# peterdavidfagan/mujoco_robot_environments

Measured on AMD Instinct MI355X. Metric: env steps/sec (whole node), RearrangementEnv batch=4096 at 1/2/4/8 MI355X, higher is better.
Workload: dtype f32

## Files before the change

mujoco_robot_environments_amd/csrc/mre_newton.h:

```cpp
#pragma once

namespace mre {

constexpr int NW_QUAD = 0, NW_SAT = 1, NW_CONE = 4;
constexpr int NW_LS_MAX = 20;
constexpr float NW_LS_TOL = 0.01f;
#ifndef NW_LS_REL_VALUE
#define NW_LS_REL_VALUE 1e-5f
#endif
constexpr float NW_LS_REL = NW_LS_REL_VALUE;

MRE_DEV float rdlane(float v, int lane) {
  return __builtin_bit_cast(float, __builtin_amdgcn_readlane(__builtin_bit_cast(int, v), lane));
}
MRE_DEV int uni(int v) { return __builtin_amdgcn_readfirstlane(v); }
MRE_DEV float unif(float v) {
  return __builtin_bit_cast(float, __builtin_amdgcn_readfirstlane(__builtin_bit_cast(int, v)));
}

MRE_DEV float nw_Jl(const Sm& s, int i, int h, int l, int lp, int lk) {
  const int rs = h & 0xFF, pa = (h >> 8) & 0xF, pb = (h >> 12) & 0xF;
  float j = 0.f;
  if (l < NRV) {
    if (rs != HDR_NONE) j = s.Jr[rs][l];
// ... 93 lines not shown
    const NwContact o = pyr ? nw_pyramid<FULL>(jar[i], jar[i + 1], jar[i + 2], D0, fr, hc)
                            : nw_contact<FULL>(jar[i], jar[i + 1], jar[i + 2], D0, D1, D2, fr, fr * mu_scale, hc);
    cost += o.cost;
    if (FULL) {
      s.frc[i] = o.f0; s.frc[i + 1] = o.f1; s.frc[i + 2] = o.f2;
      const int rs = s.con_rslot[l];
      if (rs != HDR_NONE) { s.frc_r[rs] = o.f0; s.frc_r[rs + 1] = o.f1; s.frc_r[rs + 2] = o.f2; }
      s.rstate[i] = s.rstate[i + 1] = s.rstate[i + 2] = (uint8_t)o.st;
      if (o.st == NW_CONE) {
#pragma unroll
        for (int k = 0; k < 6; k++) s.hc[l][k] = hc[k];
      }
    }
  }
  return wave_sum(cost);
}

struct NwMasks { unsigned long long sc, cq, cc; };
MRE_DEV bool operator==(const NwMasks& a, const NwMasks& b) { return a.sc == b.sc && a.cq == b.cq && a.cc == b.cc; }
MRE_DEV NwMasks nw_masks(const Sm& s, int l, int nscalar, int ncon) {
  NwMasks m;
  const int st_s = l < nscalar ? s.rstate[l] : NW_SAT;
  const int st_c = l < ncon ? s.rstate[nscalar + 3 * l] : NW_SAT;
  m.sc = __ballot(st_s == NW_QUAD);
  m.cq = __ballot(st_c == NW_QUAD);
  m.cc = __ballot(st_c == NW_CONE);
  return m;
}

MRE_DEV float nw_JTf(const Sm& s, int l, int lp, int lk, int nscalar) {
  float acc = 0.f;
  if (l < NRV) {
    const int n = s.nrrow;
    for (int rs = 0; rs < n; rs++) acc = fmaf(s.Jr[rs][l], s.frc_r[rs], acc);
  } else if (l < NV && lp < s.nprops) {
    const int n = s.ccount[lp];
    for (int t = 0; t < n; t++) {
      const int e = s.clist[lp][t], c = e & 0x7F;
      const float* J = (e & 0x80) ? s.JpB[3 * s.con_bslot[c]] : s.JpA[3 * c];
      const float* f = &s.frc[nscalar + 3 * c];
      acc = fmaf(J[lk], f[0], acc);
      acc = fmaf(J[6 + lk], f[1], acc);
      acc = fmaf(J[12 + lk], f[2], acc);
    }
  }
  return acc;
}

MRE_DEV void nw_rank1(float (&hh)[NV], float t, float J, bool has_r, int pa, int pb) {
  if (has_r) {
#pragma unroll
    for (int c = 0; c < NRV; c++) hh[c] = fmaf(t, rdlane(J, c), hh[c]);
  }
#pragma unroll
  for (int p = 0; p < NPROP; p++) {
    if (pa == p || pb == p) {
#pragma unroll
      for (int k = 0; k < 6; k++) hh[NRV + 6 * p + k] = fmaf(t, rdlane(J, NRV + 6 * p + k), hh[NRV + 6 * p + k]);
    }
  }
}

template <int HI, int LO>
MRE_DEV void nw_elim_update(float (&hh)[NV], float u) {
  constexpr int n = HI - LO + 1;
  if constexpr (n > 0) {
#pragma unroll
    for (int g0 = 0; g0 < n; g0 += 8) {
      float t[8];
#pragma unroll
      for (int q = 0; q < 8; q++)
        if (g0 + q < n) t[q] = rdlane(u, HI - g0 - q);
      __builtin_amdgcn_sched_barrier(0);
#pragma unroll
      for (int q = 0; q < 8; q++)
        if (g0 + q < n) hh[HI - g0 - q] = fmaf(-u, t[q], hh[HI - g0 - q]);
// ... 79 lines not shown
  c.lp = (l >= NRV && l < NV) ? (l - NRV) / 6 : -1;
  c.lk = (l >= NRV && l < NV) ? (l - NRV) % 6 : 0;
  c.lact = l < NRV || (c.lp >= 0 && c.lp < s.nprops);
  c.mdiag = c.lp >= 0 ? (c.lk < 3 ? s.prop_mass[c.lp] : s.prop_inertia[c.lp][c.lk - 3]) : 0.f;
  c.mu_scale = __builtin_amdgcn_rsqf(fmaxf(M->impratio, kMinVal));
  float msum = M->M0_diag_robot_sum;
  for (int p = 0; p < s.nprops; p++)
    msum += 3.f * s.prop_mass[p] + s.prop_inertia[p][0] + s.prop_inertia[p][1] + s.prop_inertia[p][2];
  c.scale = 1.0f / msum;
  return c;
}

template <bool PYR>
MRE_DEV float nw_update_gradient(Sm& s, int l, const NwLane& c, int nscalar, int ncon) {
  const float sc = nw_update<true, PYR>(s, l, nscalar, ncon, c.mu_scale, s.jar);
  MRE_SYNC();
  const float qc = nw_JTf(s, l, c.lp, c.lk, nscalar);
  const bool on = l < NV && c.lact;
  const float fs = on ? s.qfrc_smooth[l] : 0.f, as = on ? s.qacc_smooth[l] : 0.f;
  const float qa = on ? s.qacc[l] : 0.f, Ma = on ? s.nw_Ma[l] : 0.f;
  if (l < NVP) {
    s.qfrc_con[l] = on ? qc : 0.f;
    s.nw_grad[l] = on ? Ma - fs - qc : 0.f;
  }
  const float cost = sc + wave_sum(0.5f * (Ma - fs) * (qa - as));
  MRE_SYNC();
  return cost;
}

template <bool PYR>
MRE_DEV float nw_setup_impl(ModelP M, Sm& s, int l) {
  const NwLane c = nw_lane(M, s, l);
  const int nefc = s.nefc, ncon = s.ncon, nscalar = 7 + s.nl;
  for (int e = l; e < NRV * MD_LD; e += 64) (&s.Md[0][0])[e] = 0.f;
  MRE_SYNC();
  for (int e = l; e < NMR; e += 64) {
    const int i = M->M_i[e], j = M->M_j[e];
    const float v = s.qM[e];
    s.Md[i][j] = v; s.Md[j][i] = v;
  }
  MRE_SYNC();
  const bool on = l < NV && c.lact;
  const float fs = on ? s.qfrc_smooth[l] : 0.f, as = on ? s.qacc_smooth[l] : 0.f;
  float qa = on ? s.qacc[l] : 0.f;
  float Ma = on ? nw_mulM(s, l, c.mdiag, s.qacc) : 0.f;
  for (int i = l; i < nefc; i += 64) {
    const float aref = s.efc_aref[i];
    float d1, d2;
    row_dot2(s, i, s.qacc, s.qacc_smooth, d1, d2);
    s.jar[i] = d1 - aref;
    s.jv[i] = d2 - aref;
  }
  MRE_SYNC();
  const float gauss = wave_sum(0.5f * (Ma - fs) * (qa - as));
  const float cost_ws = gauss + nw_update<false, PYR>(s, l, nscalar, ncon, c.mu_scale, s.jar);
  const float cost_sm = nw_update<false, PYR>(s, l, nscalar, ncon, c.mu_scale, s.jv);
  if (cost_ws > cost_sm || !(cost_ws == cost_ws)) {
    qa = as; Ma = fs;
    for (int i = l; i < nefc; i += 64) s.jar[i] = s.jv[i];
  }
  if (l < NVP) { s.qacc[l] = qa; s.nw_Ma[l] = Ma; }
  MRE_SYNC();
  return nw_update_gradient<PYR>(s, l, c, nscalar, ncon);
}
MRE_PHASE_FN float nw_setup(ModelP M, Sm& s, int l) { return nw_setup_impl<false>(M, s, l); }
MRE_PHASE_FN float nw_setup_pyramidal(ModelP M, Sm& s, int l) { return nw_setup_impl<true>(M, s, l); }

MRE_PHASE_FN void nw_direction(ModelP M, Sm& s, int l) {
  MRE_DBG_T0();
  const NwLane c = nw_lane(M, s, l);
  const int nefc = s.nefc, nscalar = 7 + s.nl, nprops = s.nprops;
  const int lp = c.lp, lk = c.lk;
  float hh[NV];
#pragma unroll
  for (int k = 0; k < NV; k++) {
    float v = 0.f;
    if (k < NRV) { if (l < NRV) v = s.Md[l][k]; }
    else if (l == k) v = c.lact ? c.mdiag : 1.0f;
    hh[k] = v;
  }
  MRE_DBG_STAMP(4, 0);
#if defined(MRE_PHASE_STAMPS) && MRE_PHASE_STAMPS == 5
  {
    int nc_ = 0, nq_ = 0;
    for (int r0 = 0; r0 < nefc; r0 += 64) {
      const int st_ = r0 + l < nefc ? (int)s.rstate[r0 + l] : NW_SAT;
      nc_ += __popcll(__ballot(st_ == NW_CONE)); nq_ += __popcll(__ballot(st_ == NW_QUAD));
    }
    if (threadIdx.x == 0) { dbg_acc[2] += (unsigned long long)nc_ << 4; dbg_acc[3] += (unsigned long long)nq_ << 4; }
  }
#endif
  typedef float v4f __attribute__((ext_vector_type(4)));
  v4f c00 = {0.f, 0.f, 0.f, 0.f}, c10 = c00, c11 = c00, c20 = c00, c21 = c00, c22 = c00;
  {
    const int g = l >> 4, m16 = l & 15;
    const char* const sb = reinterpret_cast<const char*>(&s);
    const unsigned zoff = (unsigned)offsetof(Sm, zrow), jr0 = (unsigned)offsetof(Sm, Jr);
    const unsigned sh = m16 < 12 ? 16u * (unsigned)(m16 / 6) : 0u;
    const unsigned lo = 4u * (unsigned)(m16 % 6), lr = 4u * (unsigned)m16;
    auto ldw = [&](unsigned off) { return *reinterpret_cast<const float*>(sb + off); };
    auto meta = [&](int r0, int& ii, int& st, int& h, float& R, uint2& d) {
      const int i = r0 + g;
      ii = i < nefc ? i : 0;
      st = i < nefc ? (int)s.rstate[ii] : NW_SAT;
      h = s.hdr[ii];
      R = s.efc_R[ii];
      d = *reinterpret_cast<const uint2*>(&s.jdesc[ii][0]);
    };
    auto gather = [&](int h, uint2 d, float& w0, float& w1, float& w2) {
      const int rs = h & 0xFF;
      w0 = ldw((rs != HDR_NONE ? jr0 + 60u * (unsigned)rs : zoff) + lr);
      w1 = ldw(((d.x >> sh) & 0xFFFFu) + lo);
      w2 = nprops > 2 ? ldw(((d.y >> sh) & 0xFFFFu) + lo) : 0.f;
    };
    static_assert(sizeof(s.Jr[0]) == 60 && sizeof(s.JpA[0]) == 24 && sizeof(s.JpB[0]) == 24, "row strides of the gathers");
    struct Meta { int ii, st, h; float R; uint2 d; };
    auto chunk = [&](const Meta& cur, Meta& nxt, int r0) {
      const int ii = cur.ii, h = cur.h, st = cur.st;
      const uint2 d = cur.d;
      const bool quad = st == NW_QUAD, cone = st == NW_CONE;
      const float D = quad ? __builtin_amdgcn_rcpf(cur.R) : 0.f;
      if (r0 + 4 < nefc) meta(r0 + 4, nxt.ii, nxt.st, nxt.h, nxt.R, nxt.d);
      float v0, v1, v2, a0, a1, a2;
      if (__any(cone)) {
        const int cr = ii - nscalar;
        const int k = cone ? cr % 3 : 0;
        const int i0 = ii - k, i1 = cone ? i0 + 1 : ii, i2 = cone ? i0 + 2 : ii;
        float x0, x1, x2, y0, y1, y2, z0, z1, z2;
        gather(s.hdr[i0], *reinterpret_cast<const uint2*>(&s.jdesc[i0][0]), x0, x1, x2);
        gather(s.hdr[i1], *reinterpret_cast<const uint2*>(&s.jdesc[i1][0]), y0, y1, y2);
        gather(s.hdr[i2], *reinterpret_cast<const uint2*>(&s.jdesc[i2][0]), z0, z1, z2);
        const float* hcp = s.hc[cone ? cr / 3 : 0];
        const float H0 = k == 0 ? hcp[0] : (k == 1 ? hcp[1] : hcp[2]);
        const float H1 = k == 0 ? hcp[1] : (k == 1 ? hcp[3] : hcp[4]);
        const float H2 = k == 0 ? hcp[2] : (k == 1 ? hcp[4] : hcp[5]);
        v0 = k == 0 ? x0 : (k == 1 ? y0 : z0);
        v1 = k == 0 ? x1 : (k == 1 ? y1 : z1);
        v2 = k == 0 ? x2 : (k == 1 ? y2 : z2);
        a0 = cone ? H0 * x0 + H1 * y0 + H2 * z0 : v0 * D;
        a1 = cone ? H0 * x1 + H1 * y1 + H2 * z1 : v1 * D;
        a2 = cone ? H0 * x2 + H1 * y2 + H2 * z2 : v2 * D;
      } else {
        gather(h, d, v0, v1, v2);
        a0 = v0 * D; a1 = v1 * D; a2 = v2 * D;
      }
      c00 = __builtin_amdgcn_mfma_f32_16x16x4f32(a0, v0, c00, 0, 0, 0);
      c10 = __builtin_amdgcn_mfma_f32_16x16x4f32(a1, v0, c10, 0, 0, 0);
      c11 = __builtin_amdgcn_mfma_f32_16x16x4f32(a1, v1, c11, 0, 0, 0);
      if (nprops > 2) {
        c20 = __builtin_amdgcn_mfma_f32_16x16x4f32(a2, v0, c20, 0, 0, 0);
        c21 = __builtin_amdgcn_mfma_f32_16x16x4f32(a2, v1, c21, 0, 0, 0);
        c22 = __builtin_amdgcn_mfma_f32_16x16x4f32(a2, v2, c22, 0, 0, 0);
      }
    };
    Meta mA, mB;
    meta(0, mA.ii, mA.st, mA.h, mA.R, mA.d);
    mB = mA;
    for (int r0 = 0; r0 < nefc; r0 += 8) {
      chunk(mA, mB, r0);
      if (r0 + 4 < nefc) chunk(mB, mA, r0 + 4);
    }
    MRE_DBG_STAMP(4, 1);
    float* T = s.W;
    constexpr int TS = 17;
    const int mytile = l < NRV ? 0 : (l < NRV + 12 ? 1 : (l < NV ? 2 : -1));
    const int mym = l < NRV ? l : (l < NRV + 12 ? l - NRV : l - NRV - 12);
    auto spill = [&](const v4f& cv, int off) {
#pragma unroll
      for (int v = 0; v < 4; v++) T[off + (4 * g + v) * TS + m16] = cv[v];
    };
#define NW_TILE(OFF, TI, TJ, BI, NI, BJ, NJ)                                                   \
    if (mytile == TI) {                                                                        \
      _Pragma("unroll") for (int n = 0; n < NJ; n++) hh[BJ + n] += T[OFF + mym * TS + n];      \
    }                                                                                          \
    if (TI != TJ && mytile == TJ) {                                                            \
      _Pragma("unroll") for (int q = 0; q < NI; q++) hh[BI + q] += T[OFF + q * TS + mym];      \
    }
    constexpr int T2 = 16 * TS;
    static_assert(2 * T2 <= NV * (NV + 1) / 2, "two tiles fit the factor's storage");
    spill(c00, 0); spill(c10, T2);
    MRE_SYNC();
    NW_TILE(0, 0, 0, 0, NRV, 0, NRV)
    if (nprops > 0) { NW_TILE(T2, 1, 0, NRV, 12, 0, NRV) }
    MRE_SYNC();
    if (nprops > 0) {
      spill(c11, 0); spill(c20, T2);
      MRE_SYNC();
      NW_TILE(0, 1, 1, NRV, 12, NRV, 12)
      if (nprops > 2) { NW_TILE(T2, 2, 0, NRV + 12, 12, 0, NRV) }
      MRE_SYNC();
// ... 68 lines not shown
  float g = gin;
  const float dinv = on ? 1.0f / s.W[l * (l + 1) / 2 + l] : 1.0f;
  float y = 0.f;
  for (int k = nva - 1; k >= 0; k--) {
    const float yk = rdlane(g * dinv, k);
    const float w = (l < k) ? s.W[k * (k + 1) / 2 + l] : 0.f;
    g = fmaf(-w, yk, g);
    y = (l == k) ? yk : y;
  }
  const int base = l < NV ? l * (l + 1) / 2 : 0;
  for (int j = 0; j < nva; j++) {
    const float cw = (j < l && l < NV) ? s.W[base + j] : 0.f;
    const float xj = rdlane(y * dinv, j);
    y = fmaf(-cw, xj, y);
  }
  const float x = on ? y * dinv : 0.f;
  if (l < NVP) s.nw_search[l] = -x;
  const float dec = wave_sum(gin * x);
  if (l == 0) s.scratch[2] = dec;
  MRE_SYNC();
}

template <bool PYR>
MRE_DEV float nw_search_move_impl(ModelP M, Sm& s, int l) {
  MRE_DBG_T0();
  const NwLane c = nw_lane(M, s, l);
  const int nefc = s.nefc, ncon = s.ncon, nscalar = 7 + s.nl;
  const float tol = M->tolerance, mu_scale = c.mu_scale;
  const bool on = l < NV && c.lact;
  const float fs = on ? s.qfrc_smooth[l] : 0.f, as = on ? s.qacc_smooth[l] : 0.f;
  float qa = on ? s.qacc[l] : 0.f, Ma = on ? s.nw_Ma[l] : 0.f;
  const float sv = on ? s.nw_search[l] : 0.f;
  const float Mv = on ? nw_mulM(s, l, c.mdiag, s.nw_search) : 0.f;
  for (int i = l; i < nefc; i += 64) s.jv[i] = row_dot(s, i, s.nw_search);
  MRE_SYNC();
  MRE_DBG_STAMP(7, 0);
  const float snorm = sqrtf(wave_sum(sv * sv));
  float alpha = 0.f;
#if defined(MRE_PHASE_STAMPS) && MRE_PHASE_STAMPS == 7
  int dbg_nev = 0;
#endif
  if (snorm >= kMinVal) {
    const float gtol_abs = tol * NW_LS_TOL * snorm / c.scale;
    float g0 = 0.5f * (Ma - fs) * (qa - as), g1 = sv * (Ma - fs), g2 = 0.5f * sv * Mv;
    wave_sum3(g0, g1, g2);
    float sq0 = 0.f, sq1 = 0.f, sq2 = 0.f, sj = 0.f, svv = 0.f;
    const bool s_on = l < nscalar, s_eq = l < 7;
    if (s_on) {
      const float D = 1.0f / s.efc_R[l];
      sj = s.jar[l]; svv = s.jv[l];
      sq0 = 0.5f * D * sj * sj; sq1 = D * sj * svv; sq2 = 0.5f * D * svv * svv;
    }
    float cq0 = 0.f, cq1 = 0.f, cq2 = 0.f, U0 = 0.f, V0 = 0.f, UU = 0.f, UV = 0.f, VV = 0.f, Dm = 0.f, mu = 0.f;
    const bool c_on = l < ncon;
    constexpr bool pyr = PYR;
    float pe0 = 0.f, pe1 = 0.f, pe2 = 0.f, pe3 = 0.f, pv0 = 0.f, pv1 = 0.f, pv2 = 0.f, pv3 = 0.f, pD = 0.f;
    if (c_on && pyr) {
      const int i = nscalar + 3 * l;
      const float fr = s.con_fric[l];
      const float j0 = s.jar[i], j1 = fr * s.jar[i + 1], j2 = fr * s.jar[i + 2];
      const float v0 = s.jv[i], v1 = fr * s.jv[i + 1], v2 = fr * s.jv[i + 2];
      pe0 = j0 + j1; pe1 = j0 - j1; pe2 = j0 + j2; pe3 = j0 - j2;
      pv0 = v0 + v1; pv1 = v0 - v1; pv2 = v0 + v2; pv3 = v0 - v2;
      pD = 1.0f / s.efc_R[i];
    }
    if (c_on && !pyr) {
      const int i = nscalar + 3 * l;
// ... 250 lines not shown
        const double Dm = D[0] / fmax(mu * mu * (1.0 + mu * mu), 1e-15), NT = Nn - mu * T, iT = 1.0 / T;
        o[0] = -Dm * NT * mu;
        o[1] = -o[0] * iT * U1 * fr;
        o[2] = -o[0] * iT * U2 * fr;
        const double a = mu * Nn * iT * iT * iT, dgn = mu * mu - mu * Nn * iT;
        o[3] = Dm * mu * mu;
        o[4] = Dm * mu * fr * (-mu * U1 * iT);
        o[5] = Dm * mu * fr * (-mu * U2 * iT);
        o[6] = Dm * fr * fr * (a * U1 * U1 + dgn);
        o[7] = Dm * fr * fr * (a * U1 * U2);
        o[8] = Dm * fr * fr * (a * U2 * U2 + dgn);
      }
    }
  }
  if (l < nscalar) {
    double jar = -(double)s.efc_aref[l];
#pragma unroll
    for (int j = 0; j < NRV; j++) jar += (double)s.Jr[l][j] * (double)s.qacc[j];
    const bool act = l < 7 || s.rstate[l] == NW_QUAD;
    const double D = act ? rcp_d((double)s.efc_R[l]) : 0.0;
    frow[l] = -D * jar;
    drow[l] = D;
  }
  MRE_SYNC();
  const int d = l < NRV ? l : 0;
  const bool row = l < NRV && (full || l >= F0);
  double hrow[NRV], g = 0.0;
#pragma unroll
  for (int j = 0; j < NRV; j++) hrow[j] = row ? (double)s.Md[d][j] : 0.0;
  if (row) {
    g = -(double)s.qfrc_smooth[d];
#pragma unroll
    for (int j = 0; j < NRV; j++) g += (double)s.Md[d][j] * (double)s.qacc[j];
    for (int r = 0; r < nscalar; r++) {
      const double jd = (double)s.Jr[r][d];
      g -= jd * frow[r];
      const double t = drow[r] * jd;
      if (full) {
#pragma unroll
        for (int j = 0; j < F0; j++) hrow[j] += t * (double)s.Jr[r][j];
      }
#pragma unroll
      for (int j = F0; j < NRV; j++) hrow[j] += t * (double)s.Jr[r][j];
    }
    for (int k = 0; k < nrc; k++) {
      const double* o = fcon + 10 * k;
      const int rs = (int)o[9];
      const double j0 = (double)s.Jr[rs][d], j1 = (double)s.Jr[rs + 1][d], j2 = (double)s.Jr[rs + 2][d];
      g -= j0 * o[0] + j1 * o[1] + j2 * o[2];
      const double t0 = j0 * o[3] + j1 * o[4] + j2 * o[5], t1 = j0 * o[4] + j1 * o[6] + j2 * o[7],
                   t2 = j0 * o[5] + j1 * o[7] + j2 * o[8];
      if (full) {
#pragma unroll
        for (int j = 0; j < F0; j++)
          hrow[j] += t0 * (double)s.Jr[rs][j] + t1 * (double)s.Jr[rs + 1][j] + t2 * (double)s.Jr[rs + 2][j];
      }
#pragma unroll
      for (int j = F0; j < NRV; j++)
        hrow[j] += t0 * (double)s.Jr[rs][j] + t1 * (double)s.Jr[rs + 1][j] + t2 * (double)s.Jr[rs + 2][j];
    }
  }
  double x = -g;
  double pinv[NRV];
#pragma unroll
  for (int k = 0; k < NRV; k++) pinv[k] = 1.0;
  if (full) {
#pragma unroll
    for (int k = 0; k < F0; k++) {
      pinv[k] = rcp_d(rdlane_d(hrow[k], k));
      const double xk = rdlane_d(x, k);
      const double mlt = (l > k && l < NRV) ? hrow[k] * pinv[k] : 0.0;
#pragma unroll
      for (int j = k + 1; j < NRV; j++) hrow[j] -= mlt * rdlane_d(hrow[j], k);
      x -= mlt * xk;
    }
  }
#pragma unroll
  for (int k = F0; k < NRV; k++) {
    pinv[k] = rcp_d(rdlane_d(hrow[k], k));
    if (k == NRV - 1) break;
    const double xk = rdlane_d(x, k);
    const double mlt = (l > k && l < NRV) ? hrow[k] * pinv[k] : 0.0;
#pragma unroll
    for (int j = k + 1; j < NRV; j++) hrow[j] -= mlt * rdlane_d(hrow[j], k);
    x -= mlt * xk;
  }
#pragma unroll
  for (int k = NRV - 1; k >= F0; k--) {
    const double xk = rdlane_d(x, k) * pinv[k];
    if (l == k) x = xk;
    else if (l < k && row) x -= hrow[k] * xk;
  }
// ... 19 lines not shown
```

mujoco_robot_environments_amd/csrc/mre_solver.h:

```cpp
#pragma once

namespace mre {

constexpr int HDR_NONE = 0xFF;
constexpr int BLK_NONE = 0x7F;
constexpr int SCHED_NONE = 0xFF;
constexpr int TAB_OFF = MAXBLK * 5;
constexpr int TAB_ZEROS = 48;
static_assert(TAB_BYTES == 8 * (TAB_OFF + 1) + 4 * TAB_ZEROS, "operand table size");

#ifndef MRE_NEWTON
MRE_DEV void build_schedule(ModelP M, Sm& s);
#endif
MRE_DEV constexpr int cube_pair_bit(int p, int q) {
  const int a = p < q ? p : q, b = p < q ? q : p;
  return a == 0 ? b - 1 : (a == 1 ? b + 1 : 5);
}

MRE_DEV float prop_invM(const Sm& s, int p, int k) {
  return 1.0f / ((k < 3) ? s.prop_mass[p] : s.prop_inertia[p][k - 3]);
}

MRE_DEV void geom_pose(ModelP M, const Sm& s, int g, float* p, float* R, float* size,
                       float* rbound) {
// ... 150 lines not shown
  }
}

MRE_DEV float impedance(const float* solimp, float pos, float margin) {
  const float dmin = clampf(solimp[0], 0.0001f, 0.9999f), dmax = clampf(solimp[1], 0.0001f, 0.9999f);
  const float width = fmaxf(solimp[2], kMinVal), mid = clampf(solimp[3], 0.0001f, 0.9999f);
  const float power = fmaxf(solimp[4], 1.0f);
  if (dmin == dmax) return 0.5f * (dmin + dmax);
  const float x = fabsf((pos - margin) / width);
  if (x >= 1.0f) return dmax;
  if (x <= 0.0f) return dmin;
  float y;
  if (power == 1.0f) y = x;
  else if (power == 2.0f) {
    y = (x <= mid) ? x * x / mid : 1.0f - (1.0f - x) * (1.0f - x) / (1.0f - mid);
  }
  else if (x <= mid) y = powf(x, power) / powf(mid, power - 1.0f);
  else y = 1.0f - powf(1.0f - x, power) / powf(1.0f - mid, power - 1.0f);
  return dmin + y * (dmax - dmin);
}

MRE_DEV void jac_robot(ModelP M, Sm& s, int rs, int b, const float* p, const float* ax, float sg) {
  float off[3];
  v3sub(off, p, s.com_robot);
  const int n = M->chain_len[b];
  for (int k = 0; k < n; k++) {
    const int j = M->chain_dof[b][k];
    const float* c = s.cdof[j];
    float t[3];
    v3cross(t, c, off);
    s.Jr[rs][j] += sg * (ax[0] * (c[3] + t[0]) + ax[1] * (c[4] + t[1]) + ax[2] * (c[5] + t[2]));
  }
}
MRE_DEV int row_blk(const Sm& s, int i, int& r) {
  const int ns = 7 + s.nl;
  if (i < ns) { r = i % 3; return i / 3; }
  const int cr = i - ns;
  r = cr % 3;
  return 8 + cr / 3;
}
#ifdef MRE_NEWTON
MRE_DEV float& rowR(Sm& s, int i) { return s.efc_R[i]; }
MRE_DEV float& rowB(Sm& s, int i) { return s.efc_aref[i]; }
#else
MRE_DEV float& rowR(Sm& s, int i) { int r; const int b = row_blk(s, i, r); return s.blkrec[b][r]; }
MRE_DEV float& rowB(Sm& s, int i) { int r; const int b = row_blk(s, i, r); return s.blkrec[b][3 + r]; }
MRE_DEV float& rowAinv(Sm& s, int i) { int r; const int b = row_blk(s, i, r); return s.blkrec[b][6 + r]; }
#endif

MRE_DEV float* jpA(Sm& s, int i) { return s.JpA[i - 7 - s.nl]; }
MRE_DEV const float* jpA(const Sm& s, int i) { return s.JpA[i - 7 - s.nl]; }
MRE_DEV float* jpB(Sm& s, int i) { const int cr = i - 7 - s.nl; return s.JpB[3 * s.con_bslot[cr / 3] + cr % 3]; }
MRE_DEV const float* jpB(const Sm& s, int i) { const int cr = i - 7 - s.nl; return s.JpB[3 * s.con_bslot[cr / 3] + cr % 3]; }
MRE_DEV void jac_prop(Sm& s, int i, int slot, int b, const float* p, const float* ax, float sg) {
  float off[3];
  v3sub(off, p, s.xpos[b]);
  float* J = slot == 0 ? jpA(s, i) : jpB(s, i);
  for (int k = 0; k < 3; k++) {
    J[k] = sg * ax[k];
    float axk[3] = {s.xmat[b][k], s.xmat[b][3 + k], s.xmat[b][6 + k]}, t[3];
    v3cross(t, axk, off);
    J[3 + k] = sg * v3dot(ax, t);
  }
}

MRE_DEV float row_dot(const Sm& s, int i, const float* vec) {
  const int h = s.hdr[i];
  const int rs = h & 0xFF, pa = (h >> 8) & 0xF, pb = (h >> 12) & 0xF;
  float acc = 0.f;
  if (rs != HDR_NONE)
    for (int j = 0; j < NRV; j++) acc += s.Jr[rs][j] * vec[j];
  if (pa < NPROP)
    { const float* ja = jpA(s, i); for (int k = 0; k < 6; k++) acc += ja[k] * vec[NRV + 6 * pa + k]; }
  if (pb < NPROP)
    { const float* jb = jpB(s, i); for (int k = 0; k < 6; k++) acc += jb[k] * vec[NRV + 6 * pb + k]; }
  return acc;
}

MRE_DEV void row_dot2(const Sm& s, int i, const float* v1, const float* v2, float& r1, float& r2) {
  const int h = s.hdr[i];
  const int rs = h & 0xFF, pa = (h >> 8) & 0xF, pb = (h >> 12) & 0xF;
  float a1 = 0.f, a2 = 0.f;
  if (rs != HDR_NONE)
    for (int j = 0; j < NRV; j++) { const float jv = s.Jr[rs][j]; a1 += jv * v1[j]; a2 += jv * v2[j]; }
  if (pa < NPROP) {
    const float* ja = jpA(s, i);
    for (int k = 0; k < 6; k++) { const float jv = ja[k]; a1 += jv * v1[NRV + 6 * pa + k]; a2 += jv * v2[NRV + 6 * pa + k]; }
  }
  if (pb < NPROP) {
    const float* jb = jpB(s, i);
    for (int k = 0; k < 6; k++) { const float jv = jb[k]; a1 += jv * v1[NRV + 6 * pb + k]; a2 += jv * v2[NRV + 6 * pb + k]; }
  }
  r1 = a1; r2 = a2;
}

#ifndef MRE_NEWTON
MRE_PHASE_FN void solve_robot_rows(Sm& s, int l) {
  for (int rs = l; rs < s.nrrow; rs += 64) {
    float x[NRV];
#pragma unroll
    for (int k = 0; k < NRV; k++) x[k] = s.Jr[rs][k];
    solve_robot_regs(s.qLD, s.qLDinv, x);
#pragma unroll
    for (int k = 0; k < NRV; k++) s.Br[rs][k] = x[k];
  }
  MRE_SYNC();
}

#endif

constexpr int GRIP0 = GRIP_BODY0;

MRE_PHASE_FN void assemble_constraints(ModelP M, Sm& s, int l) {
  int lim = 0, lim_side = 0;
  const auto* BR = &M->body_rec[l < NRB ? l : 0];
  const int jnt_limited = BR->jnt_limited;
  const float jnt_range[2] = {BR->jnt_range[0], BR->jnt_range[1]};
  if (l >= 1 && l < NRB && jnt_limited) {
    const double q = robot_q(s, l - 1);
    if (q - (double)jnt_range[0] < 0.0) { lim = 1; lim_side = -1; }
    else if ((double)jnt_range[1] - q < 0.0) { lim = 1; lim_side = 1; }
  }
  keep_live(jnt_range[0]); keep_live(jnt_range[1]);
  const unsigned long long limm = __ballot(lim != 0);
  const int lim_idx = __popcll(limm & ((1ull << l) - 1ull));
  if (l == 0) s.nl = __popcll(limm);
  if (lim) s.lim_info[lim_idx] = l | ((lim_side > 0 ? 1 : 0) << 8);
// ... 37 lines not shown
      s.nefc = base + 3 * kept;
      s.nrrow = base + 3 * __popcll(rmask & below);
      s.npp = __popcll(tmask & below);
      s.finger_contact = (fingm & below) != 0ull;
#ifdef MRE_NEWTON
      s.nsched = 0; s.nblk = 0;
#else
      build_schedule(M, s);
#endif
    }
  }
  MRE_SYNC();
  const int nefc = s.nefc, nl = s.nl;
  for (int e = l; e < s.nrrow * NRV; e += 64) (&s.Jr[0][0])[e] = 0.f;
#ifndef MRE_NEWTON
  for (int e = l; e < 8 * 16; e += 64) (&s.blkrec[0][0])[e] = 0.f;
#endif
  MRE_SYNC();
  for (int i = l; i < nefc; i += 64) {
    int rs = HDR_NONE, pa = 0xF, pb = 0xF;
    float pos = 0.f, margin = 0.f, diag = 0.f, imp_pos = 0.f;
    bool fric_row = false;
    float R0scale = 1.0f;
    const int eqi = i < 6 ? i / 3 : 2;
    const int limb = (i >= 7 && i < 7 + nl) ? (s.lim_info[i - 7] & 0xFF) : 0;
    const int rrec = i < 7 ? eqi : (i < 7 + nl ? ROWREC_JNT + limb : ROWREC_PAIR + s.con_pair[(i - 7 - nl) / 3]);
    const auto* RR = &M->row_rec[rrec];
    const float solref[2] = {RR->solref[0], RR->solref[1]};
    const float solimp[5] = {RR->solimp[0], RR->solimp[1], RR->solimp[2], RR->solimp[3], RR->solimp[4]};
    const float rec_margin = RR->margin, rec_gap = RR->gap, rec_friction = RR->friction, invw1 = RR->invw1, invw2 = RR->invw2;
    const float lim_range[2] = {M->body_rec[limb].jnt_range[0], M->body_rec[limb].jnt_range[1]};
    const float opt_timestep = M->opt_rec.timestep, opt_impratio = M->opt_rec.impratio;
    const int opt_cone = M->opt_rec.cone;
    if (i < 7) {
      rs = i;
      const int e = eqi;
      const auto* E = &M->eq_rec[e];
      const int b1 = E->b1, b2 = E->b2;
      const int root = E->root, pb1 = E->pb1, pb2 = E->pb2;
      const float pc[5] = {E->data[0], E->data[1], E->data[2], E->data[3], E->data[4]};
      const float q0_1 = E->qpos0_1, q0_2 = E->qpos0_2;
      const int nchain = E->root_chain_len;
      int chain[MAXCHAIN];
#pragma unroll
      for (int c = 0; c < MAXCHAIN; c++) chain[c] = E->root_chain[c];
      if (e < 2) {
        const int k = i % 3;
        const float* loc = &s.qfrc_con[16 * e];
        const float* R = s.xmat[root];
        float cp[3];
        m3mulv(cp, R, loc);
        const float rk[3] = {R[3 * k], R[3 * k + 1], R[3 * k + 2]};
        s.Jr[rs][b1 - 1] += v3dot(rk, loc + 4);
        if (pb1 >= GRIP0) s.Jr[rs][pb1 - 1] += v3dot(rk, loc + 7);
        s.Jr[rs][b2 - 1] += v3dot(rk, loc + 10);
        if (pb2 >= GRIP0) s.Jr[rs][pb2 - 1] += v3dot(rk, loc + 13);
        {
#pragma unroll
          for (int c = 0; c < MAXCHAIN; c++) {
            if (c < nchain) {
              const int j = chain[c];
              float t[3];
              v3cross(t, s.cdof[j], cp);
              s.Jr[rs][j] += sel3(t, k);
            }
          }
        }
        pos = sel3(cp, k);
        imp_pos = v3norm(cp);
        diag = invw1 + invw2;
      } else {
        const int d1 = b1 - 1, d2 = b2 - 1;
        const double dif64 = robot_q(s, d2) - (double)q0_2;
        pos = (float)(robot_q(s, d1) - (double)q0_1 -
                      ((double)pc[0] + dif64 * ((double)pc[1] + dif64 * ((double)pc[2] + dif64 * ((double)pc[3] + dif64 * (double)pc[4])))));
        const float dif = (float)dif64;
        const float deriv = pc[1] + dif * (2.f * pc[2] + dif * (3.f * pc[3] + dif * 4.f * pc[4]));
        s.Jr[rs][d1] += 1.f;
        s.Jr[rs][d2] -= deriv;
        imp_pos = pos;
        diag = invw1 + invw2;
      }
      keep_live(root); keep_live(pb1); keep_live(pb2); keep_live(nchain); keep_live(q0_1); keep_live(q0_2);
#pragma unroll
      for (int c = 0; c < 5; c++) keep_live(pc[c]);
#pragma unroll
      for (int c = 0; c < MAXCHAIN; c++) keep_live(chain[c]);
    } else if (i < 7 + nl) {
      rs = i;
      const int info = s.lim_info[i - 7], b = info & 0xFF, hi = (info >> 8) & 1;
      const double q = robot_q(s, b - 1);
      pos = (float)(hi ? ((double)lim_range[1] - q) : (q - (double)lim_range[0]));
      s.Jr[rs][b - 1] = hi ? -1.f : 1.f;
      imp_pos = pos;
      diag = invw1;
    } else {
      const int c = (i - 7 - nl) / 3, r = (i - 7 - nl) % 3;
      const int b1 = s.con_b1[c], b2 = s.con_b2[c];
      const float* ax = &s.con_frame[c][3 * r];
      const float* p = s.con_pos[c];
      const int rs0 = s.con_rslot[c];
      if (rs0 != HDR_NONE) rs = rs0 + r;
      int slot = 0;
      float dg = 0.f;
      if (b1 > 0) {
        if (b1 < NRB) { jac_robot(M, s, rs, b1, p, ax, -1.f); dg += invw1; }
        else { pa = b1 - NRB; jac_prop(s, i, slot++, b1, p, ax, -1.f); dg += 1.0f / s.prop_mass[pa]; }
      }
      if (b2 > 0) {
        if (b2 < NRB) { jac_robot(M, s, rs, b2, p, ax, 1.f); dg += invw2; }
        else {
          const int pid = b2 - NRB;
          if (slot == 0) pa = pid; else pb = pid;
          jac_prop(s, i, slot++, b2, p, ax, 1.f);
          dg += 1.0f / s.prop_mass[pid];
        }
      }
      diag = dg;
      margin = rec_margin - rec_gap;
      imp_pos = s.con_dist[c];
      if (r == 0) pos = s.con_dist[c];
      else {
        fric_row = true;
        pos = 0.f;
        R0scale = 1.0f / fmaxf(opt_impratio, kMinVal);
      }
      if (opt_cone == 0) {
        const float fr = rec_friction;
        diag = dg * (1.f + fr * fr);
        R0scale = 2.f * fr * fr / fmaxf(opt_impratio, kMinVal);
      }
    }
    keep_live(lim_range[0]); keep_live(lim_range[1]); keep_live(invw1); keep_live(invw2); keep_live(rec_friction);
    keep_live(rec_margin); keep_live(rec_gap); keep_live(opt_impratio); keep_live(opt_cone);
    s.hdr[i] = rs | (pa << 8) | (pb << 12);
    const float imp = impedance(solimp, imp_pos, margin);
    float tc = solref[0];
    const float dr = solref[1], dmax = clampf(solimp[1], 0.0001f, 0.9999f);
    float K, B;
    if (tc > 0.f) {
      tc = fmaxf(tc, 2.f * opt_timestep);
      K = 1.0f / (dmax * dmax * tc * tc * dr * dr);
      B = 2.0f / (dmax * tc);
    } else { K = -tc / (dmax * dmax); B = -dr / dmax; }
    if (fric_row) K = 0.f;
    float R = fmaxf((1.f - imp) * diag / imp, kMinVal) * R0scale;
    if (opt_cone == 0) R = fmaxf(R, kMinVal);
    const float vel = row_dot(s, i, s.qvel);
    const float efc_margin = fric_row ? 0.f : margin;
    const float aref = -B * vel - K * imp * (pos - efc_margin);
    rowR(s, i) = R; rowB(s, i) = aref;
#ifdef MRE_NEWTON
    if (i >= 7 + nl && (i - 7 - nl) % 3 == 0) s.con_fric[(i - 7 - nl) / 3] = rec_friction;
#else
    if (i >= 7 + nl && (i - 7 - nl) % 3 == 0) s.blkrec[8 + (i - 7 - nl) / 3][15] = rec_friction;
#endif
  }
  MRE_SYNC();
}

#ifndef MRE_NEWTON
MRE_PHASE_FN void assemble_blocks(ModelP M, Sm& s, int l) {
  const int nefc = s.nefc, nl = s.nl;
  for (int i = l; i < nefc; i += 64) {
    const int h = s.hdr[i];
    const int rs = h & 0xFF, pa = (h >> 8) & 0xF, pb = (h >> 12) & 0xF;
    const bool scalar = i < 7 + nl;
    const int r = scalar ? i % 3 : (i - 7 - nl) % 3;
    const int i0 = i - r;
    const int nb = scalar ? ((7 + nl - i0) < 3 ? (7 + nl - i0) : 3) : 3;
    const int slot = scalar ? i / 3 : 8 + (i - 7 - nl) / 3;
    float acc[3] = {0.f, 0.f, 0.f};
#pragma unroll
    for (int cc = 0; cc < 3; cc++) {
      float a = 0.f;
      if (cc < nb) {
        if (rs != HDR_NONE) {
          const int rs2 = rs - r + cc;
          for (int j = 0; j < NRV; j++) a += s.Jr[rs][j] * s.Br[rs2][j];
        }
        if (pa < NPROP)
// ... 525 lines not shown
```

Measured before the change: 24.52 million.

## Batch and prefetch LDS loads across Newton solver row loops

Restructures several per-row loops in the Newton constraint solver to issue shared-memory loads ahead of use. JTf sums four rows at a time, the MFMA Hessian loop gathers the next chunk's Jacobian values one chunk early, and the double-precision Cholesky row loops are software-pipelined two deep. Row dot products now use a precomputed row descriptor with all loads hoisted before the FMAs, the Jacobian scatter in the equality rows is accumulated in registers, and the mass-matrix scatter is unrolled to two entries per lane. This aims to hide LDS latency at the cost of more registers and possible occupancy loss.

```diff
diff --git a/mujoco_robot_environments_amd/csrc/mre_newton.h b/mujoco_robot_environments_amd/csrc/mre_newton.h
--- a/mujoco_robot_environments_amd/csrc/mre_newton.h
+++ b/mujoco_robot_environments_amd/csrc/mre_newton.h
@@ -149,16 +149,56 @@
   float acc = 0.f;
   if (l < NRV) {
     const int n = s.nrrow;
-    for (int rs = 0; rs < n; rs++) acc = fmaf(s.Jr[rs][l], s.frc_r[rs], acc);
+    for (int r0 = 0; r0 < n; r0 += 4) {
+      float J[4], f[4];
+#pragma unroll
+      for (int q = 0; q < 4; q++) {
+        const int rs = r0 + q < n ? r0 + q : r0;
+        J[q] = s.Jr[rs][l]; f[q] = s.frc_r[rs];
+      }
+#pragma unroll
+      for (int q = 0; q < 4; q++)
+        if (r0 + q < n) acc = fmaf(J[q], f[q], acc);
+#pragma unroll
+      for (int q = 0; q < 4; q++) { keep_live(J[q]); keep_live(f[q]); }
+    }
   } else if (l < NV && lp < s.nprops) {
+    static_assert(offsetof(Sm, clist) % 4 == 0 && NCON_MAX % 4 == 0, "list entries read four at a time");
     const int n = s.ccount[lp];
-    for (int t = 0; t < n; t++) {
-      const int e = s.clist[lp][t], c = e & 0x7F;
-      const float* J = (e & 0x80) ? s.JpB[3 * s.con_bslot[c]] : s.JpA[3 * c];
-      const float* f = &s.frc[nscalar + 3 * c];
-      acc = fmaf(J[lk], f[0], acc);
-      acc = fmaf(J[6 + lk], f[1], acc);
-      acc = fmaf(J[12 + lk], f[2], acc);
+    const unsigned* const cl = reinterpret_cast<const unsigned*>(&s.clist[lp][0]);
+    const char* const sb = reinterpret_cast<const char*>(&s);
+    for (int t0 = 0; t0 < n; t0 += 4) {
+      const unsigned e4 = cl[t0 >> 2];
+      int row[4];
+      unsigned off[4];
+#pragma unroll
+      for (int q = 0; q < 4; q++) {
+        const int c = t0 + q < n ? (int)((e4 >> (8 * q)) & 0x7Fu) : (int)(e4 & 0x7Fu);
+        row[q] = nscalar + 3 * c;
+        off[q] = (unsigned)s.jdesc[row[q]][lp] + 4u * (unsigned)lk;
+      }
+      float J[4][3], f[4][3];
+#pragma unroll
+      for (int q = 0; q < 4; q++) {
+#pragma unroll
+        for (int r = 0; r < 3; r++) {
+          J[q][r] = *reinterpret_cast<const float*>(sb + off[q] + 24u * (unsigned)r);
+          f[q][r] = s.frc[row[q] + r];
+        }
+      }
+#pragma unroll
+      for (int q = 0; q < 4; q++) {
+        if (t0 + q < n) {
+          acc = fmaf(J[q][0], f[q][0], acc);
+          acc = fmaf(J[q][1], f[q][1], acc);
+          acc = fmaf(J[q][2], f[q][2], acc);
+        }
+      }
+#pragma unroll
+      for (int q = 0; q < 4; q++) {
+#pragma unroll
+        for (int r = 0; r < 3; r++) { keep_live(J[q][r]); keep_live(f[q][r]); }
+      }
     }
   }
   return acc;
@@ -304,13 +344,14 @@
 MRE_DEV float nw_setup_impl(ModelP M, Sm& s, int l) {
   const NwLane c = nw_lane(M, s, l);
   const int nefc = s.nefc, ncon = s.ncon, nscalar = 7 + s.nl;
+  static_assert(NMR > 64 && NMR <= 128, "two entries per lane");
+  const int e1 = l + 64 < NMR ? l + 64 : l;
+  const int mi0 = M->m_rec[l].i, mj0 = M->m_rec[l].j, mi1 = M->m_rec[e1].i, mj1 = M->m_rec[e1].j;
+  const float mv0 = s.qM[l], mv1 = s.qM[e1];
   for (int e = l; e < NRV * MD_LD; e += 64) (&s.Md[0][0])[e] = 0.f;
   MRE_SYNC();
-  for (int e = l; e < NMR; e += 64) {
-    const int i = M->M_i[e], j = M->M_j[e];
-    const float v = s.qM[e];
-    s.Md[i][j] = v; s.Md[j][i] = v;
-  }
+  s.Md[mi0][mj0] = mv0; s.Md[mj0][mi0] = mv0;
+  if (l + 64 < NMR) { s.Md[mi1][mj1] = mv1; s.Md[mj1][mi1] = mv1; }
   MRE_SYNC();
   const bool on = l < NV && c.lact;
   const float fs = on ? s.qfrc_smooth[l] : 0.f, as = on ? s.qacc_smooth[l] : 0.f;
@@ -319,7 +360,7 @@
   for (int i = l; i < nefc; i += 64) {
     const float aref = s.efc_aref[i];
     float d1, d2;
-    row_dot2(s, i, s.qacc, s.qacc_smooth, d1, d2);
+    row_dot2_parts(row_parts(s, i), s.qacc, s.qacc_smooth, d1, d2);
     s.jar[i] = d1 - aref;
     s.jv[i] = d2 - aref;
   }
@@ -386,13 +427,15 @@
       w2 = nprops > 2 ? ldw(((d.y >> sh) & 0xFFFFu) + lo) : 0.f;
     };
     static_assert(sizeof(s.Jr[0]) == 60 && sizeof(s.JpA[0]) == 24 && sizeof(s.JpB[0]) == 24, "row strides of the gathers");
-    struct Meta { int ii, st, h; float R; uint2 d; };
-    auto chunk = [&](const Meta& cur, Meta& nxt, int r0) {
+    struct Meta { int ii, st, h; float R; uint2 d; float w0, w1, w2; };
+    auto chunk = [&](Meta& cur, Meta& nxt, int r0) {
       const int ii = cur.ii, h = cur.h, st = cur.st;
       const uint2 d = cur.d;
+      const float cw0 = cur.w0, cw1 = cur.w1, cw2 = cur.w2;
       const bool quad = st == NW_QUAD, cone = st == NW_CONE;
       const float D = quad ? __builtin_amdgcn_rcpf(cur.R) : 0.f;
-      if (r0 + 4 < nefc) meta(r0 + 4, nxt.ii, nxt.st, nxt.h, nxt.R, nxt.d);
+      gather(nxt.h, nxt.d, nxt.w0, nxt.w1, nxt.w2);
+      meta(r0 + 8, cur.ii, cur.st, cur.h, cur.R, cur.d);
       float v0, v1, v2, a0, a1, a2;
       if (__any(cone)) {
         const int cr = ii - nscalar;
@@ -413,7 +456,7 @@
         a1 = cone ? H0 * x1 + H1 * y1 + H2 * z1 : v1 * D;
         a2 = cone ? H0 * x2 + H1 * y2 + H2 * z2 : v2 * D;
       } else {
-        gather(h, d, v0, v1, v2);
+        v0 = cw0; v1 = cw1; v2 = cw2;
         a0 = v0 * D; a1 = v1 * D; a2 = v2 * D;
       }
       c00 = __builtin_amdgcn_mfma_f32_16x16x4f32(a0, v0, c00, 0, 0, 0);
@@ -427,7 +470,9 @@
     };
     Meta mA, mB;
     meta(0, mA.ii, mA.st, mA.h, mA.R, mA.d);
-    mB = mA;
+    meta(4, mB.ii, mB.st, mB.h, mB.R, mB.d);
+    gather(mA.h, mA.d, mA.w0, mA.w1, mA.w2);
+    keep_live(mA.w0); keep_live(mA.w1); keep_live(mA.w2); keep_live(mB.R); keep_live((int)mB.d.x); keep_live((int)mB.d.y);
     for (int r0 = 0; r0 < nefc; r0 += 8) {
       chunk(mA, mB, r0);
       if (r0 + 4 < nefc) chunk(mB, mA, r0 + 4);
@@ -562,7 +607,7 @@
   float qa = on ? s.qacc[l] : 0.f, Ma = on ? s.nw_Ma[l] : 0.f;
   const float sv = on ? s.nw_search[l] : 0.f;
   const float Mv = on ? nw_mulM(s, l, c.mdiag, s.nw_search) : 0.f;
-  for (int i = l; i < nefc; i += 64) s.jv[i] = row_dot(s, i, s.nw_search);
+  for (int i = l; i < nefc; i += 64) s.jv[i] = row_dot_parts(row_parts(s, i), s.nw_search);
   MRE_SYNC();
   MRE_DBG_STAMP(7, 0);
   const float snorm = sqrtf(wave_sum(sv * sv));
@@ -879,20 +924,46 @@
     g = -(double)s.qfrc_smooth[d];
 #pragma unroll
     for (int j = 0; j < NRV; j++) g += (double)s.Md[d][j] * (double)s.qacc[j];
-    for (int r = 0; r < nscalar; r++) {
-      const double jd = (double)s.Jr[r][d];
-      g -= jd * frow[r];
-      const double t = drow[r] * jd;
+    struct SRow { float jd, jr[NRV]; double f, D; };
+    auto fetch_s = [&](int r, SRow& q) {
+      q.jd = s.Jr[r][d]; q.f = frow[r]; q.D = drow[r];
+#pragma unroll
+      for (int j = 0; j < NRV; j++) q.jr[j] = s.Jr[r][j];
+    };
+    auto add_s = [&](const SRow& q) {
+      const double jd = (double)q.jd;
+      g -= jd * q.f;
+      const double t = q.D * jd;
       if (full) {
 #pragma unroll
-        for (int j = 0; j < F0; j++) hrow[j] += t * (double)s.Jr[r][j];
-      }
-#pragma unroll
-      for (int j = F0; j < NRV; j++) hrow[j] += t * (double)s.Jr[r][j];
-    }
-    for (int k = 0; k < nrc; k++) {
+        for (int j = 0; j < F0; j++) hrow[j] += t * (double)q.jr[j];
+      }
+#pragma unroll
+      for (int j = F0; j < NRV; j++) hrow[j] += t * (double)q.jr[j];
+    };
+    SRow qa, qb;
+    fetch_s(0, qa);
+    for (int r = 0; r < nscalar; r += 2) {
+      fetch_s(r + 1 < nscalar ? r + 1 : r, qb);
+      add_s(qa);
+      if (r + 1 < nscalar) {
+        fetch_s(r + 2 < nscalar ? r + 2 : r + 1, qa);
+        add_s(qb);
+      }
+    }
+    struct CRow { double o[9]; int rs; };
+    auto fetch_c = [&](int k, CRow& q) {
       const double* o = fcon + 10 * k;
-      const int rs = (int)o[9];
+#pragma unroll
+      for (int t = 0; t < 9; t++) q.o[t] = o[t];
+      q.rs = (int)o[9];
+    };
+    auto add_c = [&](const CRow& q) {
+      const double* o = q.o;
+      const int rs = q.rs;
+      float r0[NRV], r1[NRV], r2[NRV];
+#pragma unroll
+      for (int j = 0; j < NRV; j++) { r0[j] = s.Jr[rs][j]; r1[j] = s.Jr[rs + 1][j]; r2[j] = s.Jr[rs + 2][j]; }
       const double j0 = (double)s.Jr[rs][d], j1 = (double)s.Jr[rs + 1][d], j2 = (double)s.Jr[rs + 2][d];
       g -= j0 * o[0] + j1 * o[1] + j2 * o[2];
       const double t0 = j0 * o[3] + j1 * o[4] + j2 * o[5], t1 = j0 * o[4] + j1 * o[6] + j2 * o[7],
@@ -900,11 +971,25 @@
       if (full) {
 #pragma unroll
         for (int j = 0; j < F0; j++)
-          hrow[j] += t0 * (double)s.Jr[rs][j] + t1 * (double)s.Jr[rs + 1][j] + t2 * (double)s.Jr[rs + 2][j];
+          hrow[j] += t0 * (double)r0[j] + t1 * (double)r1[j] + t2 * (double)r2[j];
       }
 #pragma unroll
       for (int j = F0; j < NRV; j++)
-        hrow[j] += t0 * (double)s.Jr[rs][j] + t1 * (double)s.Jr[rs + 1][j] + t2 * (double)s.Jr[rs + 2][j];
+        hrow[j] += t0 * (double)r0[j] + t1 * (double)r1[j] + t2 * (double)r2[j];
+#pragma unroll
+      for (int j = 0; j < F0; j++) { keep_live(r0[j]); keep_live(r1[j]); keep_live(r2[j]); }
+    };
+    if (nrc > 0) {
+      CRow ca, cb;
+      fetch_c(0, ca);
+      for (int k = 0; k < nrc; k += 2) {
+        fetch_c(k + 1 < nrc ? k + 1 : k, cb);
+        add_c(ca);
+        if (k + 1 < nrc) {
+          fetch_c(k + 2 < nrc ? k + 2 : k + 1, ca);
+          add_c(cb);
+        }
+      }
     }
   }
   double x = -g;
diff --git a/mujoco_robot_environments_amd/csrc/mre_solver.h b/mujoco_robot_environments_amd/csrc/mre_solver.h
--- a/mujoco_robot_environments_amd/csrc/mre_solver.h
+++ b/mujoco_robot_environments_amd/csrc/mre_solver.h
@@ -206,6 +206,10 @@
     s.Jr[rs][j] += sg * (ax[0] * (c[3] + t[0]) + ax[1] * (c[4] + t[1]) + ax[2] * (c[5] + t[2]));
   }
 }
+MRE_DEV void jr_add(float (&w)[NRV], int j, float x) {
+#pragma unroll
+  for (int q = 0; q < NRV; q++) w[q] = (q == j) ? w[q] + x : w[q];
+}
 MRE_DEV int row_blk(const Sm& s, int i, int& r) {
   const int ns = 7 + s.nl;
   if (i < ns) { r = i % 3; return i / 3; }
@@ -226,10 +230,9 @@
 MRE_DEV const float* jpA(const Sm& s, int i) { return s.JpA[i - 7 - s.nl]; }
 MRE_DEV float* jpB(Sm& s, int i) { const int cr = i - 7 - s.nl; return s.JpB[3 * s.con_bslot[cr / 3] + cr % 3]; }
 MRE_DEV const float* jpB(const Sm& s, int i) { const int cr = i - 7 - s.nl; return s.JpB[3 * s.con_bslot[cr / 3] + cr % 3]; }
-MRE_DEV void jac_prop(Sm& s, int i, int slot, int b, const float* p, const float* ax, float sg) {
+MRE_DEV void jac_prop(Sm& s, float* J, int b, const float* p, const float* ax, float sg) {
   float off[3];
   v3sub(off, p, s.xpos[b]);
-  float* J = slot == 0 ? jpA(s, i) : jpB(s, i);
   for (int k = 0; k < 3; k++) {
     J[k] = sg * ax[k];
     float axk[3] = {s.xmat[b][k], s.xmat[b][3 + k], s.xmat[b][6 + k]}, t[3];
@@ -267,6 +270,65 @@
   }
   r1 = a1; r2 = a2;
 }
+
+#ifdef MRE_NEWTON
+struct RowParts {
+  const float *jr, *ja, *jb;
+  int oa, ob;
+  bool r, a, b;
+};
+MRE_DEV RowParts row_parts(const Sm& s, int i) {
+  const int h = s.hdr[i];
+  const uint2 d = *reinterpret_cast<const uint2*>(&s.jdesc[i][0]);
+  const int rs = h & 0xFF, pa = (h >> 8) & 0xF, pb = (h >> 12) & 0xF;
+  RowParts p;
+  p.r = rs != HDR_NONE; p.a = pa < NPROP; p.b = pb < NPROP;
+  const int qa = p.a ? pa : 0, qb = p.b ? pb : 0;
+  const unsigned long long d64 = ((unsigned long long)d.y << 32) | d.x;
+  const char* const sb = reinterpret_cast<const char*>(&s);
+  p.jr = s.Jr[p.r ? rs : 0];
+  p.ja = reinterpret_cast<const float*>(sb + (unsigned)((d64 >> (16 * qa)) & 0xFFFFull));
+  p.jb = reinterpret_cast<const float*>(sb + (unsigned)((d64 >> (16 * qb)) & 0xFFFFull));
+  p.oa = NRV + 6 * qa; p.ob = NRV + 6 * qb;
+  return p;
+}
+template <int NVEC>
+MRE_DEV void row_dot_batched(const RowParts& p, const float* v1, const float* v2, float& r1, float& r2) {
+  constexpr int NW = NRV + 12;
+  float J[NW], V1[NW], V2[NW];
+#pragma unroll
+  for (int j = 0; j < NRV; j++) { J[j] = p.jr[j]; V1[j] = v1[j]; if (NVEC > 1) V2[j] = v2[j]; }
+#pragma unroll
+  for (int k = 0; k < 6; k++) {
+    J[NRV + k] = p.ja[k]; V1[NRV + k] = v1[p.oa + k]; if (NVEC > 1) V2[NRV + k] = v2[p.oa + k];
+    J[NRV + 6 + k] = p.jb[k]; V1[NRV + 6 + k] = v1[p.ob + k]; if (NVEC > 1) V2[NRV + 6 + k] = v2[p.ob + k];
+  }
+  float a1 = 0.f, a2 = 0.f;
+  if (p.r) {
+#pragma unroll
+    for (int j = 0; j < NRV; j++) { a1 += J[j] * V1[j]; if (NVEC > 1) a2 += J[j] * V2[j]; }
+  }
+  if (p.a) {
+#pragma unroll
+    for (int k = 0; k < 6; k++) { a1 += J[NRV + k] * V1[NRV + k]; if (NVEC > 1) a2 += J[NRV + k] * V2[NRV + k]; }
+  }
+  if (p.b) {
+#pragma unroll
+    for (int k = 0; k < 6; k++) { a1 += J[NRV + 6 + k] * V1[NRV + 6 + k]; if (NVEC > 1) a2 += J[NRV + 6 + k] * V2[NRV + 6 + k]; }
+  }
+#pragma unroll
+  for (int j = 0; j < NW; j++) { keep_live(J[j]); keep_live(V1[j]); if (NVEC > 1) keep_live(V2[j]); }
+  r1 = a1; r2 = a2;
+}
+MRE_DEV float row_dot_parts(const RowParts& p, const float* vec) {
+  float r1, r2;
+  row_dot_batched<1>(p, vec, vec, r1, r2);
+  return r1;
+}
+MRE_DEV void row_dot2_parts(const RowParts& p, const float* v1, const float* v2, float& r1, float& r2) {
+  row_dot_batched<2>(p, v1, v2, r1, r2);
+}
+#endif
 
 #ifndef MRE_NEWTON
 MRE_PHASE_FN void solve_robot_rows(Sm& s, int l) {
@@ -370,9 +432,18 @@
     const float lim_range[2] = {M->body_rec[limb].jnt_range[0], M->body_rec[limb].jnt_range[1]};
     const float opt_timestep = M->opt_rec.timestep, opt_impratio = M->opt_rec.impratio;
     const int opt_cone = M->opt_rec.cone;
+    const bool is_con = i >= 7 + nl;
+    const int rc = is_con ? (i - 7 - nl) / 3 : 0, rr = is_con ? (i - 7 - nl) % 3 : 0;
+    const int c_b1 = s.con_b1[rc], c_b2 = s.con_b2[rc], c_rslot = s.con_rslot[rc], c_bslot = s.con_bslot[rc];
+    const float c_dist = s.con_dist[rc];
+    const float c_ax[3] = {s.con_frame[rc][3 * rr], s.con_frame[rc][3 * rr + 1], s.con_frame[rc][3 * rr + 2]};
+    const float c_p[3] = {s.con_pos[rc][0], s.con_pos[rc][1], s.con_pos[rc][2]};
     if (i < 7) {
       rs = i;
       const int e = eqi;
+      float jw[NRV];
+#pragma unroll
+      for (int j = 0; j < NRV; j++) jw[j] = 0.f;
       const auto* E = &M->eq_rec[e];
       const int b1 = E->b1, b2 = E->b2;
       const int root = E->root, pb1 = E->pb1, pb2 = E->pb2;
@@ -389,10 +460,10 @@
         float cp[3];
         m3mulv(cp, R, loc);
         const float rk[3] = {R[3 * k], R[3 * k + 1], R[3 * k + 2]};
-        s.Jr[rs][b1 - 1] += v3dot(rk, loc + 4);
-        if (pb1 >= GRIP0) s.Jr[rs][pb1 - 1] += v3dot(rk, loc + 7);
-        s.Jr[rs][b2 - 1] += v3dot(rk, loc + 10);
-        if (pb2 >= GRIP0) s.Jr[rs][pb2 - 1] += v3dot(rk, loc + 13);
+        jr_add(jw, b1 - 1, v3dot(rk, loc + 4));
+        if (pb1 >= GRIP0) jr_add(jw, pb1 - 1, v3dot(rk, loc + 7));
+        jr_add(jw, b2 - 1, v3dot(rk, loc + 10));
+        if (pb2 >= GRIP0) jr_add(jw, pb2 - 1, v3dot(rk, loc + 13));
         {
 #pragma unroll
           for (int c = 0; c < MAXCHAIN; c++) {
@@ -400,7 +471,7 @@
               const int j = chain[c];
               float t[3];
               v3cross(t, s.cdof[j], cp);
-              s.Jr[rs][j] += sel3(t, k);
+              jr_add(jw, j, sel3(t, k));
             }
           }
         }
@@ -414,11 +485,13 @@
                       ((double)pc[0] + dif64 * ((double)pc[1] + dif64 * ((double)pc[2] + dif64 * ((double)pc[3] + dif64 * (double)pc[4])))));
         const float dif = (float)dif64;
         const float deriv = pc[1] + dif * (2.f * pc[2] + dif * (3.f * pc[3] + dif * 4.f * pc[4]));
-        s.Jr[rs][d1] += 1.f;
-        s.Jr[rs][d2] -= deriv;
+        jr_add(jw, d1, 1.f);
+        jr_add(jw, d2, -deriv);
         imp_pos = pos;
         diag = invw1 + invw2;
       }
+#pragma unroll
+      for (int j = 0; j < NRV; j++) s.Jr[rs][j] = jw[j];
       keep_live(root); keep_live(pb1); keep_live(pb2); keep_live(nchain); keep_live(q0_1); keep_live(q0_2);
 #pragma unroll
       for (int c = 0; c < 5; c++) keep_live(pc[c]);
@@ -433,31 +506,34 @@
       imp_pos = pos;
       diag = invw1;
     } else {
-      const int c = (i - 7 - nl) / 3, r = (i - 7 - nl) % 3;
-      const int b1 = s.con_b1[c], b2 = s.con_b2[c];
-      const float* ax = &s.con_frame[c][3 * r];
-      const float* p = s.con_pos[c];
-      const int rs0 = s.con_rslot[c];
+      const int r = rr;
+      const int b1 = c_b1, b2 = c_b2;
+      const float* ax = c_ax;
+      const float* p = c_p;
+      const int rs0 = c_rslot;
       if (rs0 != HDR_NONE) rs = rs0 + r;
+      float* const JA = s.JpA[i - 7 - nl];
+      float* const JB = s.JpB[3 * c_bslot + r];
       int slot = 0;
       float dg = 0.f;
       if (b1 > 0) {
         if (b1 < NRB) { jac_robot(M, s, rs, b1, p, ax, -1.f); dg += invw1; }
-        else { pa = b1 - NRB; jac_prop(s, i, slot++, b1, p, ax, -1.f); dg += 1.0f / s.prop_mass[pa]; }
+        else { pa = b1 - NRB; jac_prop(s, JA, b1, p, ax, -1.f); slot++; dg += 1.0f / s.prop_mass[pa]; }
       }
       if (b2 > 0) {
         if (b2 < NRB) { jac_robot(M, s, rs, b2, p, ax, 1.f); dg += invw2; }
         else {
           const int pid = b2 - NRB;
           if (slot == 0) pa = pid; else pb = pid;
-          jac_prop(s, i, slot++, b2, p, ax, 1.f);
+          jac_prop(s, slot == 0 ? JA : JB, b2, p, ax, 1.f);
+          slot++;
           dg += 1.0f / s.prop_mass[pid];
         }
       }
       diag = dg;
       margin = rec_margin - rec_gap;
-      imp_pos = s.con_dist[c];
-      if (r == 0) pos = s.con_dist[c];
+      imp_pos = c_dist;
+      if (r == 0) pos = c_dist;
       else {
         fric_row = true;
         pos = 0.f;
@@ -484,7 +560,17 @@
     if (fric_row) K = 0.f;
     float R = fmaxf((1.f - imp) * diag / imp, kMinVal) * R0scale;
     if (opt_cone == 0) R = fmaxf(R, kMinVal);
+#ifdef MRE_NEWTON
+    RowParts rp;
+    rp.r = rs != HDR_NONE; rp.a = pa < NPROP; rp.b = pb < NPROP;
+    rp.jr = s.Jr[rp.r ? rs : 0];
+    rp.ja = s.JpA[is_con ? i - 7 - nl : 0];
+    rp.jb = s.JpB[is_con ? 3 * c_bslot + rr : 0];
+    rp.oa = NRV + 6 * (rp.a ? pa : 0); rp.ob = NRV + 6 * (rp.b ? pb : 0);
+    const float vel = row_dot_parts(rp, s.qvel);
+#else
     const float vel = row_dot(s, i, s.qvel);
+#endif
     const float efc_margin = fric_row ? 0.f : margin;
     const float aref = -B * vel - K * imp * (pos - efc_margin);
     rowR(s, i) = R; rowB(s, i) = aref;
```

Result: no change. 24.45 million, median of 2 (-0.3%).
